# brdav/refign

Measured on AMD Instinct MI355X. Metric: image-pairs/s (align+seg fwd+bwd, 1080x1920), higher is better.
Workload: dtype bf16

## Files before the change

include/refign_hip.h:

```cpp
#ifndef REFIGN_HIP_H
#define REFIGN_HIP_H

#ifdef __cplusplus
extern "C" {
#endif

#define RFN_OK 0
#define RFN_EINVAL (-1)
#define RFN_ELAUNCH (-2)
#define RFN_ENOTSUP (-3)
#define RFN_ENONDET (-4)

#define RFN_ABI_VERSION 5

typedef void* rfn_stream_t;

int rfn_abi_version(void);
const char* rfn_last_error(void);

int rfn_set_deterministic(int on);
int rfn_get_deterministic(void);

int rfn_corr_fwd_f32(const float* in1, const float* in2, float* out, int B, int C, int iH, int iW,
                     int kH, int kW, int patchH, int patchW, int padH, int padW, int dilH, int dilW,
// ... 42 lines not shown
int rfn_maxpool2x2_nhwc16(const void* x, void* y, int B, int H, int W, int C, int dtype, rfn_stream_t stream);
int rfn_retile_copy(const void* src, void* dst, int B, int h, int w, int k, int units16, int src_stride16, int backward,
                    rfn_stream_t stream);

unsigned long rfn_refine_workspace_bytes(int B);
int rfn_refine_f32(const float* logits_trg, const float* logits_ref, const unsigned char* warp_mask,
                   const float* certs, float* out, void* workspace, int B, int C, int H, int W, float gamma,
                   int flags, rfn_stream_t stream);

int rfn_label_majority(const long* gt, long* out, int B, int H, int W, int scale, int n_classes, int ignore_index,
                       float min_ratio, rfn_stream_t stream);

int rfn_align_tail_f32(const float* logits_ref, const float* flow_q, const float* logvar_q, float* warped,
                       unsigned char* mask, float* cert, float* flow_up, int B, int C, int H, int W, int h,
                       int w, rfn_stream_t stream);

int rfn_dwconv3x3_nhwc_fwd(const void* x, const float* weight, const float* bias, void* y, int B, int H, int W,
                           int C, int dilation, int dtype, int flip, rfn_stream_t stream);
int rfn_dwconv3x3_nhwc_fwd_stats(const void* x, const float* weight, const float* bias, void* y, double* sums, int B, int H,
                                 int W, int C, int dilation, int dtype, rfn_stream_t stream);
int rfn_dwconv3x3_nhwc_stats(const void* x, const float* weight, const float* bias, double* sums, int B, int H, int W, int C,
                             int dilation, int dtype, rfn_stream_t stream);
int rfn_dwconv3x3_bn_act_nhwc_fwd(const void* x, const float* weight, const float* bias, const float* gamma, const float* beta,
                                  const double* sums, float* running_mean, float* running_var, void* y, int B, int H, int W,
                                  int C, int dilation, float eps, float momentum, int relu, int dtype, rfn_stream_t stream);

int rfn_dwconv3x3_gelu_nhwc_fwd(const void* x, const float* weight, const float* bias, void* y_pre, void* y_act, int B,
                                int H, int W, int C, int dtype, rfn_stream_t stream);
unsigned long rfn_dwconv3x3_bwd_weight_workspace_bytes(int C);
int rfn_dwconv3x3_nhwc_bwd_weight(const void* x, const void* grad_y, float* grad_weight, float* grad_bias,
// ... 302 lines not shown
```

refign_amd/csrc/bilinear.h:

```cpp
#pragma once
#include <hip/hip_runtime.h>

namespace rfn {

struct WarpTap {
  int o00, o01, o10, o11;
  float w00, w01, w10, w11;
  bool inside;
  float tx, ty;
  bool v00, v01, v10, v11;
  bool finite;
};

__device__ __forceinline__ WarpTap warp_tap(float gx, float gy, float fx, float fy, int H, int W) {
#pragma clang fp contract(off)
  const float wm = (float)max(W - 1, 1), hm = (float)max(H - 1, 1);
  const float vx = 2.0f * (gx + fx) / wm - 1.0f;
  const float vy = 2.0f * (gy + fy) / hm - 1.0f;
  const float ix = ((vx + 1.0f) / 2.0f) * (float)(W - 1);
  const float iy = ((vy + 1.0f) / 2.0f) * (float)(H - 1);
  float x0f = floorf(ix), y0f = floorf(iy);
  WarpTap t;
  t.tx = ix - x0f;
  t.ty = iy - y0f;
  x0f = fminf(fmaxf(x0f, -2.0f), (float)W);
  y0f = fminf(fmaxf(y0f, -2.0f), (float)H);
  if (!(ix == ix) || !(iy == iy)) { x0f = -2.0f; y0f = -2.0f; }
  const int x0 = (int)x0f, y0 = (int)y0f, x1 = x0 + 1, y1 = y0 + 1;
  const bool vx0 = x0 >= 0 && x0 < W, vx1 = x1 >= 0 && x1 < W;
  const bool vy0 = y0 >= 0 && y0 < H, vy1 = y1 >= 0 && y1 < H;
  const int cx0 = min(max(x0, 0), W - 1), cx1 = min(max(x1, 0), W - 1);
  const int cy0 = min(max(y0, 0), H - 1), cy1 = min(max(y1, 0), H - 1);
  t.o00 = cy0 * W + cx0; t.o01 = cy0 * W + cx1; t.o10 = cy1 * W + cx0; t.o11 = cy1 * W + cx1;
  t.v00 = vx0 && vy0; t.v01 = vx1 && vy0; t.v10 = vx0 && vy1; t.v11 = vx1 && vy1;
  const float ax = 1.0f - t.tx, ay = 1.0f - t.ty;
  t.w00 = t.v00 ? ax * ay : 0.0f;
  t.w01 = t.v01 ? t.tx * ay : 0.0f;
  t.w10 = t.v10 ? ax * t.ty : 0.0f;
  t.w11 = t.v11 ? t.tx * t.ty : 0.0f;
  t.inside = (vx > -1.0f) && (vy > -1.0f) && (vx < 1.0f) && (vy < 1.0f);
  t.finite = (ix == ix) && (iy == iy) && fabsf(ix) < 1e9f && fabsf(iy) < 1e9f;
  return t;
}

__device__ __forceinline__ float tap_sample(const float* __restrict__ src, const WarpTap& t) {
#pragma clang fp contract(off)
  return src[t.o00] * t.w00 + src[t.o01] * t.w01 + src[t.o10] * t.w10 + src[t.o11] * t.w11;
}

template <bool CLAMP>
__device__ __forceinline__ void up_split(float s, int in, int& i0, int& i1, float& l1) {
  if constexpr (CLAMP) {
    i0 = min((int)s, in - 1);
    i1 = i0 + (i0 < in - 1 ? 1 : 0);
  } else {
    i0 = (int)s;
    i1 = min(i0 + 1, in - 1);
  }
  l1 = s - (float)i0;
}
template <bool CLAMP = true>
__device__ __forceinline__ void up_src(int dst, float scale, int in, int& i0, int& i1, float& l1) {
  up_split<CLAMP>(fmaxf(scale * ((float)dst + 0.5f) - 0.5f, 0.f), in, i0, i1, l1);
}
__device__ __forceinline__ void up_src_nofma(int dst, float scale, int in, int& i0, int& i1, float& l1) {
  float s;
  {
#pragma clang fp contract(off)
    s = scale * ((float)dst + 0.5f) - 0.5f;
  }
  up_split<true>(fmaxf(s, 0.f), in, i0, i1, l1);
}

__device__ __forceinline__ void up_cell_window(int cell, float scale, int out_size, int& lo, int& hi) {
  const float inv = 1.f / scale;
  lo = cell <= 1 ? 0 : max(0, (int)floorf(((float)cell - 0.5f) * inv - 0.5f) - 1);
  hi = min(out_size, (int)ceilf(((float)cell + 1.5f) * inv - 0.5f) + 2);
}

}
```

refign_amd/csrc/refine.hip:

```cpp
#include "common.h"

namespace rfn {

constexpr int kClasses = 19;
constexpr int kPartials = 256;

__device__ __forceinline__ bool is_static_large(int c) {
  return (c <= 4) || (c >= 8 && c <= 10);
}

__global__ __launch_bounds__(256) void refine_entropy_kernel(const float* __restrict__ logits,
                                                             double* __restrict__ partials, int HW) {
  const int n = blockIdx.y;
  const float* p = logits + (size_t)n * kClasses * HW;
  double local = 0.0;
  for (int pix = blockIdx.x * 256 + threadIdx.x; pix < HW; pix += kPartials * 256) {
    float v[kClasses];
    float m = -INFINITY;
#pragma unroll
    for (int c = 0; c < kClasses; ++c) {
      v[c] = p[(size_t)c * HW + pix];
      m = fmaxf(m, v[c]);
    }
    float sum = 0.0f;
#pragma unroll
    for (int c = 0; c < kClasses; ++c) {
      v[c] -= m;
      sum += expf(v[c]);
    }
    const float lsum = logf(sum);
    float ent = 0.0f;
#pragma unroll
    for (int c = 0; c < kClasses; ++c) {
      const float lp = v[c] - lsum;
      ent -= (expf(v[c]) / sum) * lp;
    }
    local += (double)ent;
  }
  __shared__ double red[4];
#pragma unroll
  for (int o = 32; o > 0; o >>= 1) local += __shfl_xor(local, o, 64);
  if ((threadIdx.x & 63) == 0) red[threadIdx.x >> 6] = local;
  __syncthreads();
  if (threadIdx.x == 0) partials[(size_t)n * kPartials + blockIdx.x] = red[0] + red[1] + red[2] + red[3];
}

__global__ __launch_bounds__(256) void refine_blend_kernel(const float* __restrict__ lt, const float* __restrict__ lr,
                                                           const unsigned char* __restrict__ wmask,
                                                           const float* __restrict__ certs, float* __restrict__ out,
                                                           const double* __restrict__ partials, int HW, float gamma,
                                                           int flags) {
  const int n = blockIdx.y;
  __shared__ double red[4];
  __shared__ float s_trust;
  {
    double v = partials[(size_t)n * kPartials + threadIdx.x];
#pragma unroll
    for (int o = 32; o > 0; o >>= 1) v += __shfl_xor(v, o, 64);
    if ((threadIdx.x & 63) == 0) red[threadIdx.x >> 6] = v;
    __syncthreads();
    if (threadIdx.x == 0) {
      const double mean_ent = (red[0] + red[1] + red[2] + red[3]) / (double)HW;
      const float eta_mean = (float)(mean_ent / log((double)kClasses));
      s_trust = powf(eta_mean, gamma);
    }
    __syncthreads();
  }
  const float s = s_trust;
  const int pix = blockIdx.x * 256 + threadIdx.x;
  if (pix >= HW) return;
  const float* pt = lt + (size_t)n * kClasses * HW + pix;
  const float* pr = lr + (size_t)n * kClasses * HW + pix;
  float a[kClasses], b[kClasses];
  float ma = -INFINITY, mb = -INFINITY;
#pragma unroll
  for (int c = 0; c < kClasses; ++c) {
    a[c] = pt[(size_t)c * HW];
    b[c] = pr[(size_t)c * HW];
    ma = fmaxf(ma, a[c]);
    mb = fmaxf(mb, b[c]);
  }
  float sa = 0.0f, sb = 0.0f;
#pragma unroll
  for (int c = 0; c < kClasses; ++c) {
    a[c] = expf(a[c] - ma);
    b[c] = expf(b[c] - mb);
    sa += a[c];
    sb += b[c];
  }
  int ia = 0, ib = 0;
  float pa = -1.0f, pb = -1.0f;
#pragma unroll
  for (int c = 0; c < kClasses; ++c) {
    a[c] = a[c] / sa;
    b[c] = b[c] / sb;
    if (a[c] > pa) { pa = a[c]; ia = c; }
    if (b[c] > pb) { pb = b[c]; ib = c; }
  }
  const bool M = !(flags & 1) && is_static_large(ia) && is_static_large(ib);
  const float P = (certs != nullptr && !(flags & 2)) ? certs[(size_t)n * HW + pix] : 0.5f;
  const bool valid = (wmask == nullptr) || (wmask[(size_t)n * HW + pix] != 0);
  float* po = out + (size_t)n * kClasses * HW + pix;
#pragma unroll
  for (int c = 0; c < kClasses; ++c) {
    const float mc = (M && is_static_large(c)) ? 1.0f : 0.0f;
    const float eps = valid ? s * fmaxf(P, mc) : 0.0f;
    po[(size_t)c * HW] = (1.0f - eps) * a[c] + eps * b[c];
  }
}

__global__ __launch_bounds__(64) void label_majority_kernel(const long* __restrict__ gt, long* __restrict__ out, int H,
                                                            int W, int oh, int ow, int scale, int n_classes, int ignore,
                                                            float min_ratio) {
  const int cell = blockIdx.x, n = blockIdx.y, lane = threadIdx.x;
  const int cy = cell / ow, cx = cell % ow;
  const int y0 = cy * scale, x0 = cx * scale;
  const int hh = min(scale, H - y0), ww = min(scale, W - x0);
  const long* g = gt + (size_t)n * H * W;
  const int nb = n_classes + 1;
  int cnt[33];
#pragma unroll
  for (int c = 0; c < 33; ++c) cnt[c] = 0;
  for (int i = lane; i < hh * ww; i += 64) {
// ... 57 lines not shown
```

refign_amd/csrc/warp.hip:

```cpp
#include "bilinear.h"
#include "common.h"

namespace rfn {

template <int CG>
__global__ __launch_bounds__(256) void warp_kernel(const float* __restrict__ x, const float* __restrict__ flow,
                                                   float* __restrict__ out, unsigned char* __restrict__ mask,
                                                   int C, int H, int W) {
  const int pix = blockIdx.x * 256 + threadIdx.x;
  const int HW = H * W;
  if (pix >= HW) return;
  const int n = blockIdx.z, c0 = blockIdx.y * CG;
  const int gy = pix / W, gx = pix - gy * W;
  const float* fl = flow + (size_t)n * 2 * HW;
  const WarpTap t = warp_tap((float)gx, (float)gy, fl[pix], fl[HW + pix], H, W);
  if (mask != nullptr && blockIdx.y == 0) mask[(size_t)n * HW + pix] = t.inside ? 1 : 0;
  const float* src = x + ((size_t)n * C + c0) * HW;
  float* dst = out + ((size_t)n * C + c0) * HW + pix;
  const int cend = min(CG, C - c0);
  for (int c = 0; c < cend; ++c) dst[(size_t)c * HW] = tap_sample(src + (size_t)c * HW, t);
}

__device__ __forceinline__ int det_exponent(unsigned bits) { return max((int)(bits >> 23), 1) - 126; }
__device__ __forceinline__ double pow2(int e) { return __longlong_as_double((long long)(1023 + e) << 52); }
// ... 96 lines not shown
  const long idx = (long)blockIdx.x * 256 + threadIdx.x;
  if (idx < nx) {
    const unsigned mb = maxbits[idx / HW];
    float v = 0.0f;
    if (mb >= 0x7f800000u) v = __uint_as_float(0x7fc00000u);
    else if (mb != 0u) v = (float)((double)acc[idx] * pow2(det_exponent(mb) - F));
    gx_out[idx] = v;
  } else if (idx < nx + nf) {
    const long j = idx - nx;
    float s = 0.0f;
    for (int g = 0; g < G; ++g) s += part[(size_t)g * nf + j];
    gflow[j] = s;
  }
}

__device__ __forceinline__ float up_sample(const float* __restrict__ p, int w, int y0, int y1, int x0, int x1,
                                           float ly0, float ly1, float lx0, float lx1) {
#pragma clang fp contract(off)
  return ly0 * (lx0 * p[y0 * w + x0] + lx1 * p[y0 * w + x1]) + ly1 * (lx0 * p[y1 * w + x0] + lx1 * p[y1 * w + x1]);
}

__global__ __launch_bounds__(256) void align_tail_kernel(const float* __restrict__ logits,
                                                         const float* __restrict__ flow_q,
                                                         const float* __restrict__ logvar_q,
                                                         float* __restrict__ warped, unsigned char* __restrict__ mask,
                                                         float* __restrict__ cert, float* __restrict__ flow_up, int C,
                                                         int H, int W, int h, int w, float sy, float sx) {
  const int pix = blockIdx.x * 256 + threadIdx.x;
  const int HW = H * W, hw = h * w;
  if (pix >= HW) return;
  const int n = blockIdx.z;
  const int gy = pix / W, gx = pix - gy * W;
  int y0, y1, x0, x1;
  float ly1, lx1;
  up_src_nofma(gy, sy, h, y0, y1, ly1);
  up_src_nofma(gx, sx, w, x0, x1, lx1);
// ... 125 lines not shown
```

refign_amd/graphs.py:

```python
import contextlib
import gc
import os
import warnings

import torch


def enabled():
    return os.environ.get("RFN_HIP_GRAPH", "1") != "0"


def concurrent_stream(device, peers, priority=0, tries=8, spin_cycles=4_000_000):
    cur = torch.cuda.current_stream(device)

    def span(streams):
        start, end = torch.cuda.Event(enable_timing=True), torch.cuda.Event(enable_timing=True)
        start.record(cur)
        for st in streams:
            if st != cur:
                st.wait_event(start)
            with torch.cuda.stream(st):
                torch.cuda._sleep(spin_cycles)
        for st in streams:
            if st != cur:
# ... 40 lines not shown
    if isinstance(out, (list, tuple)):
        return type(out)(_fresh_containers(o) for o in out)
    return out


class GraphedNoGrad:
    def __init__(self, fn, name, warmup=1):
        self.fn, self.name, self.warmup = fn, name, warmup
        self.generation = 0
        self.states = {}

    def reset(self):
        self.generation += 1
        self.states.clear()

    def __call__(self, *tensors):
        if not tensors[0].is_cuda or not enabled() or torch.is_grad_enabled() or \
                torch.cuda.is_current_stream_capturing():
            return self.fn(*tensors)
        key = (tuple((tuple(t.shape), t.dtype, t.device) for t in tensors), torch.is_autocast_enabled("cuda"),
               torch.get_autocast_dtype("cuda"), self.generation)
        st = self.states.get(key)
        if st is None:
            st = self.states[key] = {"calls": 0, "graph": None, "failed": False}
        if st["failed"]:
            return self.fn(*tensors)
        if st["graph"] is None:
            st["calls"] += 1
            if st["calls"] <= self.warmup:
                return self.fn(*tensors)
            try:
                self._capture(st, tensors)
            except Exception as e:
                st["failed"] = True
                warnings.warn(f"refign_amd.graphs: capture of '{self.name}' failed ({type(e).__name__}: {e}); "
                              f"running it eagerly")
                torch.cuda.synchronize()
                return self.fn(*tensors)
        for s, t in zip(st["inputs"], tensors):
            s.copy_(t)
        st["graph"].replay()
        return _fresh_containers(st["outputs"])

    def _capture(self, st, tensors):
        inputs = [t.clone() for t in tensors]
        cur = torch.cuda.current_stream()
        side = torch.cuda.Stream()
        side.wait_stream(cur)
        with torch.cuda.stream(side):
            self.fn(*inputs)
        cur.wait_stream(side)
        torch.cuda.synchronize()
        g = torch.cuda.CUDAGraph()
        try:
            with _no_cyclic_gc(), torch.cuda.graph(g, capture_error_mode="thread_local"):
                outputs = self.fn(*inputs)
        except BaseException:
            torch.cuda.set_stream(cur)
            raise
        st["graph"], st["inputs"], st["outputs"] = g, inputs, outputs


class GraphedStep:

    def __init__(self, fn, name, warmup=2, shared=None, capture_context=None, after_capture=None, on_replay=None,
                 before_capture=None):
        self.fn, self.name, self.warmup = fn, name, warmup
        self.capture_context = capture_context
        self.after_capture, self.on_replay = after_capture, on_replay
        self.before_capture = before_capture
        self._last = None
# ... 307 lines not shown
```

refign_amd/refine.py:

```python
import torch

from . import _lib
from ._tensor import ptr, require_device_tensor, same_device


@torch.no_grad()
def refine(logits_trg, logits_ref, warp_mask, certs, gamma=0.25, disable_M=False, disable_P=False):
    logits_trg = require_device_tensor(logits_trg.float().contiguous(), "logits_trg", torch.float32)
    logits_ref = require_device_tensor(logits_ref.float().contiguous(), "logits_ref", torch.float32)
    dev = same_device(logits_trg, logits_ref, warp_mask, certs)
    B, C, H, W = logits_trg.shape
    assert C == 19, 'we assume cityscapes classes'
    if logits_ref.shape != logits_trg.shape:
        raise RuntimeError("refine: logits_trg / logits_ref shape mismatch")
    m8 = None
    if warp_mask is not None:
        if tuple(warp_mask.shape) != (B, H, W):
            raise RuntimeError("refine: warp_mask must be (B,H,W)")
        m8 = warp_mask.contiguous()
        m8 = m8.view(torch.uint8) if m8.dtype == torch.bool else m8.to(torch.uint8)
    if certs is not None:
        certs = require_device_tensor(certs.float().contiguous(), "certs", torch.float32)
        if certs.numel() != B * H * W:
            raise RuntimeError("refine: certs must be (B,1,H,W)")
    lib = _lib.load_library()
    ws = torch.empty(lib.rfn_refine_workspace_bytes(B), dtype=torch.uint8, device=dev)
    out = torch.empty_like(logits_trg)
    flags = (1 if disable_M else 0) | (2 if disable_P else 0)
    _lib.call("rfn_refine_f32", dev, ptr(logits_trg), ptr(logits_ref), ptr(m8), ptr(certs), ptr(out), ptr(ws), B, C, H, W,
              float(gamma), flags)
    return out
```

refign_amd/uda.py:

```python
import contextlib
import copy
import math
import os
import random
from typing import Optional, Sequence

import numpy as np
import torch
import torch.nn as nn
import torch.nn.functional as F

from . import align as align_mod
from . import refine as refine_mod
from ._tensor import const_tensor, upload_async
from . import dacs as _dacs
from . import f8 as _f8
from .graphs import GraphedNoGrad, GraphedSegment, GraphedSplitStep, GraphedStep
from .params import ema_update
from .upsample import interpolate_bilinear
from .config import instantiate_class
from . import seg as _seg
from .seg import DeviceBox, defer_logits, draw_crop_offsets, hrda_backbone, hrda_head, predraw_crop, push_device_crop

IMNET_MEAN = (0.485, 0.456, 0.406)
# ... 93 lines not shown

def _upsample_logits(logits, size):
    if logits.is_cuda:
        logits = logits.contiguous()
    return interpolate_bilinear(logits, size=size)


def _logits_for_loss(model, logits, size):
    return defer_logits(logits, size, _seg.fused_ce_consumer(model))


_ALIGN_PREFETCH = True
_MERGE_FD_BACKWARD = True
_EARLY_MIXED_FWD = True
_SRC_BWD_AFTER_TEACHER = True
_SIDE_PRIORITY = 0


class DomainAdaptationSegmentationModel(nn.Module):

    def __init__(self,
                 optimizer_init: dict,
                 lr_scheduler_init: dict,
                 backbone: nn.Module,
                 head: nn.Module,
                 loss: nn.Module,
                 alignment_backbone: Optional[nn.Module] = None,
                 alignment_head: Optional[nn.Module] = None,
                 metrics: dict = {},
                 backbone_lr_factor: float = 1.0,
# ... 395 lines not shown

    def _training_step_graphed(self, batch, images_src, gt_src, src_classes, opt, sch):
        ready = torch.cuda.current_stream().record_event() if self._overlap_teacher(images_src) else None
        off = self._crop_offsets(images_src, "src")
        cur = torch.cuda.current_stream()
        feat_next = self._take_imnet_prefetch(images_src) if self.enable_fdist else None
        src_graph, mix_graph = self._graphs["source_pass"], self._graphs["mixed_pass"]
        src_graph.forward(images_src, off, variant=feat_next is not None)
        src_fwd_done = cur.record_event()
        mix = early = None
        hold = _SRC_BWD_AFTER_TEACHER and ready is not None
        if hold:
            mix = self._mixed_stream(images_src)
            if mix is not None:
                mix.wait_event(ready)
            early = self._start_target_branch(batch, images_src, after=ready)
            if mix is not None:
                cur.wait_stream(self._side_stream)
        if feat_next is not None:
            feat_next = feat_next.clone()
            prefetch_free = cur.record_event()
            losses = src_graph.backward(images_src, gt_src, feat_next)
        else:
            losses = src_graph.backward(images_src, gt_src)
            prefetch_free = cur.record_event()
        if not hold:
            mix = self._mixed_stream(images_src) if ready is not None else None
            if mix is not None:
                mix.wait_event(ready)
            early = None if ready is None else self._start_target_branch(batch, images_src, after=ready)
        self.log("train_loss_src", losses[0])
        if self.enable_fdist:
            self.log("train_loss_featdist_src", losses[1])
        if early is None:
            mix = None
        run_on = cur if mix is None else mix
        if mix is not None and getattr(self, "_grad_buffer", None) is not None:
            self._grad_buffer.reduce_first_now()
        nb = batch['image_trg'].shape[0]
        src_nb, gt_nb = (images_src[:nb], gt_src[:nb]) if images_src.shape[0] > nb else (images_src, gt_src)
        early_fwd = (_EARLY_MIXED_FWD and mix is not None and self._dacs_kernels_usable(src_nb, early[0], gt_nb))
        if mix is not None:
            self.__dict__["_mixed_concurrent_steps"] = self.__dict__.get("_mixed_concurrent_steps", 0) + 1
            if early_fwd:
                mix.wait_event(src_fwd_done)
# ... 48 lines not shown
        if src_graph.any_failed() != mix_graph.any_failed():
            (mix_graph if src_graph.any_failed() else src_graph).give_up()
        opt.step()
        sch.step()
        self.global_step += 1

    def _prefetch_next(self, batch, prefetch_free, branch_done, with_flow, stream):
        nxt = batch.get("image_src_next")
        if nxt is not None:
            self.prefetch_imnet_features(nxt, after=prefetch_free, stream=stream)
        if batch.get("image_trg_next") is not None and batch.get("image_ref_next") is not None and with_flow \
                and self._next_step_aligns(batch["image_src"]):
            with torch.no_grad():
                self.prefetch_align_flow(batch["image_ref_next"], batch["image_trg_next"], after=branch_done, stream=stream)

    @torch.no_grad()
    def _target_branch(self, batch):
        if self.adapt_to_ref and random.random() < 0.5:
            adapt_to_ref, images_trg = True, batch['image_ref']
        else:
            adapt_to_ref, images_trg = False, batch['image_trg']
        if self.use_refign and not adapt_to_ref:
            return images_trg, self._teacher_align_refine(images_trg, batch['image_ref'])
        m_logits_trg = self.m_head(self._graphs["teacher_backbone"](images_trg))
        m_logits_trg = _upsample_logits(m_logits_trg, images_trg.shape[-2:])
        self.__dict__["_adapted_to_ref_steps"] = self.__dict__.get("_adapted_to_ref_steps", 0) + int(adapt_to_ref)
        return images_trg, F.softmax(m_logits_trg, dim=1)

    def _overlap_teacher(self, x):
        return x.is_cuda

    def _start_target_branch(self, batch, images_src, after=None):
        self._ensure_side_stream(images_src.device)
        if after is not None:
            self._side_stream.wait_event(after)
        else:
            if self.adapt_to_ref and self.use_hrda and self.training:
                H, W = images_src.shape[-2:]
                predraw_crop(H, W, (int(H * 0.5), int(W * 0.5)), self.hrda_output_stride * 2.0)
            self._side_stream.wait_stream(torch.cuda.current_stream())
        with torch.cuda.stream(self._side_stream):
            return self._target_branch(batch)

    def _ensure_side_stream(self, device):
        if getattr(self, "_side_stream", None) is None or self._side_stream.device != device:
            if _SIDE_PRIORITY == 0:
                from .graphs import concurrent_stream
                with torch.cuda.device(device):
                    self._side_stream, self._side_stream_probe = concurrent_stream(device, [torch.cuda.current_stream(device)])
                return
            self._side_stream = torch.cuda.Stream(device=device, priority=_SIDE_PRIORITY)

    def _teacher_align_refine(self, images_trg, images_ref):
        b = images_trg.shape[0]
        m_input = torch.cat((images_trg, images_ref))
        m_logits = self.m_head(self._graphs["teacher_backbone"](m_input))
        m_logits = _upsample_logits(m_logits, m_input.shape[-2:])
        m_logits_trg, m_logits_ref = torch.split(m_logits, [b, b], dim=0)
        if self.use_align:
            if self._align_split(images_trg):
                flow = self._take_align_prefetch(images_ref, images_trg)
                if flow is None:
                    flow = self._graphs["align_flow"](images_ref, images_trg)
                return self._graphs["tail_refine"](m_logits_trg.contiguous(), m_logits_ref.contiguous(), *flow)
            return self._graphs["align_refine"](m_logits_trg.contiguous(), m_logits_ref.contiguous(), images_ref,
                                                images_trg)
        return self.refine(m_logits_trg, m_logits_ref, None, None)

    def _align_refine(self, logits_trg, logits_ref, images_ref, images_trg):
        warped, warp_mask, warp_certs = self.align(logits_ref, images_ref, images_trg)
        return self.refine(logits_trg, warped, warp_mask, warp_certs)

    def _align_flow(self, images_ref, images_trg):
        return align_mod.align_flow(self.alignment_backbone, self.alignment_head, images_ref, images_trg)

    def _tail_refine(self, logits_trg, logits_ref, flow_q, logvar_q):
        warped, warp_mask, warp_certs = align_mod.align_from_flow(logits_ref, flow_q, logvar_q)
        return self.refine(logits_trg, warped, warp_mask, warp_certs)

    def _align_split(self, x):
        return _ALIGN_PREFETCH and self.use_refign and self.use_align and x.is_cuda and self._overlap_teacher(x)

    def _next_step_aligns(self, images_src):
        if not self.adapt_to_ref:
            return True
        state = random.getstate()
        try:
            if self.use_hrda:
                H, W = images_src.shape[-2:]
                draw_crop_offsets(H, W, (int(H * 0.5), int(W * 0.5)), self.hrda_output_stride * 2.0)
            return not random.random() < 0.5
# ... 198 lines not shown
                  'color_jitter_p': self.color_jitter_p, 'blur': random.uniform(0, 1) if self.blur else 0}
        classes = torch.unique(gt_src) if src_classes is None else src_classes
        bits = _dacs.draw_class_bits(classes, nb)
        jit, sig = [], []
        for i in range(nb):
            jit.append(_dacs.draw_jitter(self.color_jitter_s) if params['color_jitter'] > params['color_jitter_p']
                       else None)
            sig.append(np.random.uniform(0.15, 1.15) if params['blur'] > 0.5 else None)
        return {"bits": bits, "jitter": jit, "sigma": sig}

    def _dacs_kernels_usable(self, images_src, images_trg, gt_src):
        return os.environ.get("RFN_DACS_KERNEL", "1") != "0" and _dacs.usable(
            images_src, images_trg, gt_src, getattr(getattr(self, "head", None), "num_classes", 19))

    def _pseudo_labels(self, probs_trg):
        pseudo_prob, pseudo_label = torch.max(probs_trg, dim=1)
        weight = (pseudo_prob >= self.pseudo_label_threshold).sum() / pseudo_label.numel()
        pseudo_weight = torch.full_like(pseudo_prob, 1.0) * weight
        if self.psweight_ignore_top > 0:
            pseudo_weight[:, :self.psweight_ignore_top, :] = 0
        if self.psweight_ignore_bottom > 0:
            pseudo_weight[:, -self.psweight_ignore_bottom:, :] = 0
        return pseudo_label, pseudo_weight

    @torch.no_grad()
    def get_dacs_mix(self, images_trg, probs_trg, images_src, gt_src, src_classes=None):
        nb = images_trg.shape[0]
        if images_src.shape[0] > nb:
            images_src, gt_src = images_src[:nb], gt_src[:nb]
        cls = DomainAdaptationSegmentationModel
        if cls._dacs_kernels_usable(self, images_src, images_trg, gt_src):
# ... 131 lines not shown
```

Before: 17.48.

## Fuse teacher upsample, warp, refine and pseudo-label argmax into a low-res tail kernel

Adds a teacher-tail kernel pair that reads low-resolution teacher logits and flow directly. It bilinearly upsamples them on the fly, computes entropy-based trust, warps the reference logits, blends them and optionally emits only the per-pixel max probability and label. This avoids materialising full-resolution upsampled logits, warped logits and the full probability tensor before torch.max. The cost is more complex nested interpolation arithmetic per pixel and a risk of numerical differences from the original op order.

Result: no change. 17.62 (median of 6 runs) (+0.8%).

```diff
diff --git a/include/refign_hip.h b/include/refign_hip.h
--- a/include/refign_hip.h
+++ b/include/refign_hip.h
@@ -80,6 +80,11 @@
 int rfn_align_tail_f32(const float* logits_ref, const float* flow_q, const float* logvar_q, float* warped,
                        unsigned char* mask, float* cert, float* flow_up, int B, int C, int H, int W, int h,
                        int w, rfn_stream_t stream);
+
+int rfn_teacher_tail_f32(const float* logits_trg, const float* logits_ref, long stride_b, long stride_c, long stride_y,
+                         long stride_x, const float* flow_q, const float* logvar_q, void* workspace, float* probs,
+                         float* pseudo_prob, long* pseudo_label, unsigned char* mask, float* cert, int B, int C, int h, int w,
+                         int hf, int wf, int H, int W, float gamma, int flags, rfn_stream_t stream);
 
 int rfn_dwconv3x3_nhwc_fwd(const void* x, const float* weight, const float* bias, void* y, int B, int H, int W,
                            int C, int dilation, int dtype, int flip, rfn_stream_t stream);
diff --git a/refign_amd/csrc/bilinear.h b/refign_amd/csrc/bilinear.h
--- a/refign_amd/csrc/bilinear.h
+++ b/refign_amd/csrc/bilinear.h
@@ -10,6 +10,7 @@
   float tx, ty;
   bool v00, v01, v10, v11;
   bool finite;
+  int cx0, cx1, cy0, cy1;
 };
 
 __device__ __forceinline__ WarpTap warp_tap(float gx, float gy, float fx, float fy, int H, int W) {
@@ -31,6 +32,7 @@
   const bool vy0 = y0 >= 0 && y0 < H, vy1 = y1 >= 0 && y1 < H;
   const int cx0 = min(max(x0, 0), W - 1), cx1 = min(max(x1, 0), W - 1);
   const int cy0 = min(max(y0, 0), H - 1), cy1 = min(max(y1, 0), H - 1);
+  t.cx0 = cx0; t.cx1 = cx1; t.cy0 = cy0; t.cy1 = cy1;
   t.o00 = cy0 * W + cx0; t.o01 = cy0 * W + cx1; t.o10 = cy1 * W + cx0; t.o11 = cy1 * W + cx1;
   t.v00 = vx0 && vy0; t.v01 = vx1 && vy0; t.v10 = vx0 && vy1; t.v11 = vx1 && vy1;
   const float ax = 1.0f - t.tx, ay = 1.0f - t.ty;
@@ -43,9 +45,12 @@
   return t;
 }
 
+__device__ __forceinline__ float tap_combine(float nw, float ne, float sw, float se, const WarpTap& t) {
+#pragma clang fp contract(off)
+  return nw * t.w00 + ne * t.w01 + sw * t.w10 + se * t.w11;
+}
 __device__ __forceinline__ float tap_sample(const float* __restrict__ src, const WarpTap& t) {
-#pragma clang fp contract(off)
-  return src[t.o00] * t.w00 + src[t.o01] * t.w01 + src[t.o10] * t.w10 + src[t.o11] * t.w11;
+  return tap_combine(src[t.o00], src[t.o01], src[t.o10], src[t.o11], t);
 }
 
 template <bool CLAMP>
@@ -72,6 +77,15 @@
   up_split<true>(fmaxf(s, 0.f), in, i0, i1, l1);
 }
 
+__device__ __forceinline__ float up_lerp(float l0, float a, float l1, float b) {
+#pragma clang fp contract(off)
+  return l0 * a + l1 * b;
+}
+__device__ __forceinline__ float up_sample(const float* __restrict__ p, int w, int y0, int y1, int x0, int x1,
+                                           float ly0, float ly1, float lx0, float lx1) {
+  return up_lerp(ly0, up_lerp(lx0, p[y0 * w + x0], lx1, p[y0 * w + x1]), ly1, up_lerp(lx0, p[y1 * w + x0], lx1, p[y1 * w + x1]));
+}
+
 __device__ __forceinline__ void up_cell_window(int cell, float scale, int out_size, int& lo, int& hi) {
   const float inv = 1.f / scale;
   lo = cell <= 1 ? 0 : max(0, (int)floorf(((float)cell - 0.5f) * inv - 0.5f) - 1);
diff --git a/refign_amd/csrc/refine.hip b/refign_amd/csrc/refine.hip
--- a/refign_amd/csrc/refine.hip
+++ b/refign_amd/csrc/refine.hip
@@ -1,13 +1,7 @@
 #include "common.h"
+#include "refine_px.h"
 
 namespace rfn {
-
-constexpr int kClasses = 19;
-constexpr int kPartials = 256;
-
-__device__ __forceinline__ bool is_static_large(int c) {
-  return (c <= 4) || (c >= 8 && c <= 10);
-}
 
 __global__ __launch_bounds__(256) void refine_entropy_kernel(const float* __restrict__ logits,
                                                              double* __restrict__ partials, int HW) {
@@ -16,33 +10,11 @@
   double local = 0.0;
   for (int pix = blockIdx.x * 256 + threadIdx.x; pix < HW; pix += kPartials * 256) {
     float v[kClasses];
-    float m = -INFINITY;
 #pragma unroll
-    for (int c = 0; c < kClasses; ++c) {
-      v[c] = p[(size_t)c * HW + pix];
-      m = fmaxf(m, v[c]);
-    }
-    float sum = 0.0f;
-#pragma unroll
-    for (int c = 0; c < kClasses; ++c) {
-      v[c] -= m;
-      sum += expf(v[c]);
-    }
-    const float lsum = logf(sum);
-    float ent = 0.0f;
-#pragma unroll
-    for (int c = 0; c < kClasses; ++c) {
-      const float lp = v[c] - lsum;
-      ent -= (expf(v[c]) / sum) * lp;
-    }
-    local += (double)ent;
+    for (int c = 0; c < kClasses; ++c) v[c] = p[(size_t)c * HW + pix];
+    local += (double)pixel_entropy(v);
   }
-  __shared__ double red[4];
-#pragma unroll
-  for (int o = 32; o > 0; o >>= 1) local += __shfl_xor(local, o, 64);
-  if ((threadIdx.x & 63) == 0) red[threadIdx.x >> 6] = local;
-  __syncthreads();
-  if (threadIdx.x == 0) partials[(size_t)n * kPartials + blockIdx.x] = red[0] + red[1] + red[2] + red[3];
+  store_entropy_partial(local, partials, n);
 }
 
 __global__ __launch_bounds__(256) void refine_blend_kernel(const float* __restrict__ lt, const float* __restrict__ lr,
@@ -51,62 +23,23 @@
                                                            const double* __restrict__ partials, int HW, float gamma,
                                                            int flags) {
   const int n = blockIdx.y;
-  __shared__ double red[4];
-  __shared__ float s_trust;
-  {
-    double v = partials[(size_t)n * kPartials + threadIdx.x];
-#pragma unroll
-    for (int o = 32; o > 0; o >>= 1) v += __shfl_xor(v, o, 64);
-    if ((threadIdx.x & 63) == 0) red[threadIdx.x >> 6] = v;
-    __syncthreads();
-    if (threadIdx.x == 0) {
-      const double mean_ent = (red[0] + red[1] + red[2] + red[3]) / (double)HW;
-      const float eta_mean = (float)(mean_ent / log((double)kClasses));
-      s_trust = powf(eta_mean, gamma);
-    }
-    __syncthreads();
-  }
-  const float s = s_trust;
+  const float s = trust_score(partials, n, HW, gamma);
   const int pix = blockIdx.x * 256 + threadIdx.x;
   if (pix >= HW) return;
   const float* pt = lt + (size_t)n * kClasses * HW + pix;
   const float* pr = lr + (size_t)n * kClasses * HW + pix;
   float a[kClasses], b[kClasses];
-  float ma = -INFINITY, mb = -INFINITY;
 #pragma unroll
   for (int c = 0; c < kClasses; ++c) {
     a[c] = pt[(size_t)c * HW];
     b[c] = pr[(size_t)c * HW];
-    ma = fmaxf(ma, a[c]);
-    mb = fmaxf(mb, b[c]);
   }
-  float sa = 0.0f, sb = 0.0f;
-#pragma unroll
-  for (int c = 0; c < kClasses; ++c) {
-    a[c] = expf(a[c] - ma);
-    b[c] = expf(b[c] - mb);
-    sa += a[c];
-    sb += b[c];
-  }
-  int ia = 0, ib = 0;
-  float pa = -1.0f, pb = -1.0f;
-#pragma unroll
-  for (int c = 0; c < kClasses; ++c) {
-    a[c] = a[c] / sa;
-    b[c] = b[c] / sb;
-    if (a[c] > pa) { pa = a[c]; ia = c; }
-    if (b[c] > pb) { pb = b[c]; ib = c; }
-  }
-  const bool M = !(flags & 1) && is_static_large(ia) && is_static_large(ib);
   const float P = (certs != nullptr && !(flags & 2)) ? certs[(size_t)n * HW + pix] : 0.5f;
   const bool valid = (wmask == nullptr) || (wmask[(size_t)n * HW + pix] != 0);
+  refine_pixel(a, b, s, P, valid, flags);
   float* po = out + (size_t)n * kClasses * HW + pix;
 #pragma unroll
-  for (int c = 0; c < kClasses; ++c) {
-    const float mc = (M && is_static_large(c)) ? 1.0f : 0.0f;
-    const float eps = valid ? s * fmaxf(P, mc) : 0.0f;
-    po[(size_t)c * HW] = (1.0f - eps) * a[c] + eps * b[c];
-  }
+  for (int c = 0; c < kClasses; ++c) po[(size_t)c * HW] = a[c];
 }
 
 __global__ __launch_bounds__(64) void label_majority_kernel(const long* __restrict__ gt, long* __restrict__ out, int H,
diff --git a/refign_amd/csrc/refine_px.h b/refign_amd/csrc/refine_px.h
--- /dev/null
+++ b/refign_amd/csrc/refine_px.h
@@ -0,0 +1,92 @@
+#pragma once
+#include "common.h"
+
+namespace rfn {
+
+constexpr int kClasses = 19;
+constexpr int kPartials = 256;
+
+__device__ __forceinline__ bool is_static_large(int c) {
+  return (c <= 4) || (c >= 8 && c <= 10);
+}
+
+__device__ __forceinline__ float pixel_entropy(float (&v)[kClasses]) {
+  float m = -INFINITY;
+#pragma unroll
+  for (int c = 0; c < kClasses; ++c) m = fmaxf(m, v[c]);
+  float sum = 0.0f;
+#pragma unroll
+  for (int c = 0; c < kClasses; ++c) {
+    v[c] -= m;
+    sum += expf(v[c]);
+  }
+  const float lsum = logf(sum);
+  float ent = 0.0f;
+#pragma unroll
+  for (int c = 0; c < kClasses; ++c) {
+    const float lp = v[c] - lsum;
+    ent -= (expf(v[c]) / sum) * lp;
+  }
+  return ent;
+}
+
+__device__ __forceinline__ void store_entropy_partial(double local, double* __restrict__ partials, int n) {
+  __shared__ double red[4];
+#pragma unroll
+  for (int o = 32; o > 0; o >>= 1) local += __shfl_xor(local, o, 64);
+  if ((threadIdx.x & 63) == 0) red[threadIdx.x >> 6] = local;
+  __syncthreads();
+  if (threadIdx.x == 0) partials[(size_t)n * kPartials + blockIdx.x] = red[0] + red[1] + red[2] + red[3];
+}
+
+__device__ __forceinline__ float trust_score(const double* __restrict__ partials, int n, int HW, float gamma) {
+  __shared__ double red[4];
+  __shared__ float s_trust;
+  double v = partials[(size_t)n * kPartials + threadIdx.x];
+#pragma unroll
+  for (int o = 32; o > 0; o >>= 1) v += __shfl_xor(v, o, 64);
+  if ((threadIdx.x & 63) == 0) red[threadIdx.x >> 6] = v;
+  __syncthreads();
+  if (threadIdx.x == 0) {
+    const double mean_ent = (red[0] + red[1] + red[2] + red[3]) / (double)HW;
+    const float eta_mean = (float)(mean_ent / log((double)kClasses));
+    s_trust = powf(eta_mean, gamma);
+  }
+  __syncthreads();
+  return s_trust;
+}
+
+__device__ __forceinline__ void refine_pixel(float (&a)[kClasses], float (&b)[kClasses], float s, float P, bool valid, int flags) {
+  float ma = -INFINITY, mb = -INFINITY;
+#pragma unroll
+  for (int c = 0; c < kClasses; ++c) {
+    ma = fmaxf(ma, a[c]);
+    mb = fmaxf(mb, b[c]);
+  }
+  float sa = 0.0f, sb = 0.0f;
+#pragma unroll
+  for (int c = 0; c < kClasses; ++c) {
+    a[c] = expf(a[c] - ma);
+    b[c] = expf(b[c] - mb);
+    sa += a[c];
+    sb += b[c];
+  }
+  int ia = 0, ib = 0;
+  float pa = -1.0f, pb = -1.0f;
+#pragma unroll
+  for (int c = 0; c < kClasses; ++c) {
+    a[c] = a[c] / sa;
+    b[c] = b[c] / sb;
+    if (a[c] > pa) { pa = a[c]; ia = c; }
+    if (b[c] > pb) { pb = b[c]; ib = c; }
+  }
+  const bool M = !(flags & 1) && is_static_large(ia) && is_static_large(ib);
+#pragma unroll
+  for (int c = 0; c < kClasses; ++c) {
+    const float mc = (M && is_static_large(c)) ? 1.0f : 0.0f;
+    const float eps = valid ? s * fmaxf(P, mc) : 0.0f;
+    a[c] = (1.0f - eps) * a[c] + eps * b[c];
+  }
+}
+
+}
diff --git a/refign_amd/csrc/teachertail.hip b/refign_amd/csrc/teachertail.hip
--- /dev/null
+++ b/refign_amd/csrc/teachertail.hip
@@ -0,0 +1,271 @@
+#include "bilinear.h"
+#include "common.h"
+#include "refine_px.h"
+
+namespace rfn {
+
+constexpr int kTtT = 16;
+constexpr int kTtS = 20;
+constexpr int kTtF = 10;
+
+struct TtStrides {
+  long b, c, y, x;
+};
+
+constexpr int kTtGroups = 5;
+__device__ __forceinline__ constexpr int tt_group_first(int j) { return j < kTtGroups - 1 ? 4 * j : kClasses - 4; }
+typedef float tt_float4 __attribute__((ext_vector_type(4), aligned(4)));
+
+template <bool CL>
+__device__ __forceinline__ void tt_load4(const float* __restrict__ p, long sc, int c0, float (&v)[4]) {
+  if constexpr (CL) {
+    const tt_float4 q = *reinterpret_cast<const tt_float4*>(p + c0);
+    v[0] = q.x, v[1] = q.y, v[2] = q.z, v[3] = q.w;
+  } else {
+#pragma unroll
+    for (int k = 0; k < 4; ++k) v[k] = p[(c0 + k) * sc];
+  }
+}
+
+struct TtPixel {
+  float q[4][kTtGroups][4];
+  float ly0, ly1, lx0, lx1;
+};
+template <bool CL>
+__device__ __forceinline__ void tt_pixel_load(const float* __restrict__ p, const TtStrides& st, int pix, int W, int h, int w,
+                                              float sy, float sx, TtPixel& t) {
+  const long sc = CL ? 1 : st.c;
+  const int gy = pix / W, gx = pix - gy * W;
+  int y0, y1, x0, x1;
+  up_src(gy, sy, h, y0, y1, t.ly1);
+  up_src(gx, sx, w, x0, x1, t.lx1);
+  t.ly0 = 1.0f - t.ly1, t.lx0 = 1.0f - t.lx1;
+  const float* cell[4] = {p + y0 * st.y + x0 * st.x, p + y0 * st.y + x1 * st.x, p + y1 * st.y + x0 * st.x, p + y1 * st.y + x1 * st.x};
+#pragma unroll
+  for (int j = 0; j < kTtGroups; ++j)
+#pragma unroll
+    for (int i = 0; i < 4; ++i) tt_load4<CL>(cell[i], sc, tt_group_first(j), t.q[i][j]);
+}
+__device__ __forceinline__ void tt_pixel_blend(const TtPixel& t, float (&v)[kClasses]) {
+#pragma unroll
+  for (int j = 0; j < kTtGroups; ++j) {
+    const int c0 = tt_group_first(j);
+#pragma unroll
+    for (int k = 4 * j - c0; k < 4; ++k)
+      v[c0 + k] = up_lerp(t.ly0, up_lerp(t.lx0, t.q[0][j][k], t.lx1, t.q[1][j][k]), t.ly1,
+                          up_lerp(t.lx0, t.q[2][j][k], t.lx1, t.q[3][j][k]));
+  }
+}
+
+template <bool CL>
+__global__ __launch_bounds__(256) void tail_entropy_kernel(const float* __restrict__ lt, TtStrides st,
+                                                           double* __restrict__ partials, int H, int W, int h, int w,
+                                                           float sy, float sx) {
+  const int n = blockIdx.y, HW = H * W;
+  const float* p = lt + (size_t)n * st.b;
+  double local = 0.0;
+  for (long pix = blockIdx.x * 256 + threadIdx.x; pix < HW; pix += 2 * kPartials * 256) {
+    const long pix1 = pix + kPartials * 256;
+    const bool has1 = pix1 < HW;
+    TtPixel t0, t1;
+    tt_pixel_load<CL>(p, st, (int)pix, W, h, w, sy, sx, t0);
+    tt_pixel_load<CL>(p, st, has1 ? (int)pix1 : HW - 1, W, h, w, sy, sx, t1);
+    float v0[kClasses], v1[kClasses];
+    tt_pixel_blend(t0, v0);
+    tt_pixel_blend(t1, v1);
+    local += (double)pixel_entropy(v0);
+    const float e1 = pixel_entropy(v1);
+    local += has1 ? (double)e1 : 0.0;
+  }
+  store_entropy_partial(local, partials, n);
+}
+
+template <bool CL>
+__global__ __launch_bounds__(256) void tail_refine_kernel(const float* __restrict__ lt, const float* __restrict__ lr, TtStrides st,
+                                                          const float* __restrict__ flow_q, const float* __restrict__ logvar_q,
+                                                          const double* __restrict__ partials, float* __restrict__ probs,
+                                                          float* __restrict__ pseudo_prob, long* __restrict__ pseudo_label,
+                                                          unsigned char* __restrict__ mask, float* __restrict__ cert, int H, int W,
+                                                          int h, int w, int hf, int wf, float sy, float sx, float sfy, float sfx,
+                                                          float gamma, int flags) {
+  __shared__ __attribute__((aligned(16))) float lo[kTtF * kTtF * kTtS];
+  const int n = blockIdx.z, tid = threadIdx.x;
+  const int HW = H * W;
+  const long sc = CL ? 1 : st.c;
+  const float s = trust_score(partials, n, HW, gamma);
+
+  const int Y0 = blockIdx.y * kTtT, X0 = blockIdx.x * kTtT;
+  int fy0, fx0, nfy, nfx;
+  {
+    int i0, i1;
+    float l;
+    up_src(Y0, sy, h, fy0, i1, l);
+    up_src(min(Y0 + kTtT, H) - 1, sy, h, i0, i1, l);
+    nfy = min(i1 - fy0 + 1, kTtF);
+    up_src(X0, sx, w, fx0, i1, l);
+    up_src(min(X0 + kTtT, W) - 1, sx, w, i0, i1, l);
+    nfx = min(i1 - fx0 + 1, kTtF);
+  }
+  const float* pt = lt + (size_t)n * st.b;
+  for (int i = tid; i < nfy * nfx * kTtGroups; i += 256) {
+    const int q = i / kTtGroups, c0 = tt_group_first(i - q * kTtGroups);
+    const int fy = q / nfx, fx = q - fy * nfx;
+    float v[4];
+    tt_load4<CL>(pt + (fy0 + fy) * st.y + (fx0 + fx) * st.x, sc, c0, v);
+#pragma unroll
+    for (int k = 0; k < 4; ++k) lo[q * kTtS + c0 + k] = v[k];
+  }
+  __syncthreads();
+
+  const int gy = Y0 + tid / kTtT, gx = X0 + tid % kTtT;
+  if (gy >= H || gx >= W) return;
+  const int pix = gy * W + gx;
+
+  float P;
+  WarpTap t;
+  {
+    int y0, y1, x0, x1;
+    float ly1, lx1;
+    up_src_nofma(gy, sfy, hf, y0, y1, ly1);
+    up_src_nofma(gx, sfx, wf, x0, x1, lx1);
+    const float ly0 = 1.0f - ly1, lx0 = 1.0f - lx1;
+    const int hwf = hf * wf;
+    const float* fq = flow_q + (size_t)n * 2 * hwf;
+    const float fx = up_sample(fq, wf, y0, y1, x0, x1, ly0, ly1, lx0, lx1);
+    const float fy = up_sample(fq + hwf, wf, y0, y1, x0, x1, ly0, ly1, lx0, lx1);
+    const float lv = up_sample(logvar_q + (size_t)n * hwf, wf, y0, y1, x0, x1, ly0, ly1, lx0, lx1);
+    P = 1.0f - expf(-1.0f / (2.0f * expf(lv)));
+    t = warp_tap((float)gx, (float)gy, fx, fy, H, W);
+  }
+  if (cert != nullptr) cert[(size_t)n * HW + pix] = P;
+  if (mask != nullptr) mask[(size_t)n * HW + pix] = t.inside ? 1 : 0;
+  if (flags & 2) P = 0.5f;
+
+  float b[kClasses];
+  {
+    int ya0, ya1, yb0, yb1, xa0, xa1, xb0, xb1;
+    float lya1, lyb1, lxa1, lxb1;
+    up_src(t.cy0, sy, h, ya0, ya1, lya1);
+    up_src(t.cy1, sy, h, yb0, yb1, lyb1);
+    up_src(t.cx0, sx, w, xa0, xa1, lxa1);
+    up_src(t.cx1, sx, w, xb0, xb1, lxb1);
+    const float lya0 = 1.0f - lya1, lyb0 = 1.0f - lyb1, lxa0 = 1.0f - lxa1, lxb0 = 1.0f - lxb1;
+    const bool same_y = yb0 == ya0, same_x = xb0 == xa0;
+    const float* pr = lr + (size_t)n * st.b;
+    int cell[3][3];
+#pragma unroll
+    for (int j = 0; j < 3; ++j)
+#pragma unroll
+      for (int i = 0; i < 3; ++i) cell[j][i] = (int)(min(ya0 + j, h - 1) * st.y + min(xa0 + i, w - 1) * st.x);
+    float rr[2][3][3][4];
+#pragma unroll
+    for (int j = 0; j < 3; ++j)
+#pragma unroll
+      for (int i = 0; i < 3; ++i) tt_load4<CL>(pr + cell[j][i], sc, 0, rr[0][j][i]);
+#pragma unroll
+    for (int g = 0; g < kTtGroups; ++g) {
+      const int c0 = tt_group_first(g);
+      if (g + 1 < kTtGroups) {
+        if (g > 0)
+          asm volatile("" : "+v"(cell[0][0]), "+v"(cell[0][1]), "+v"(cell[0][2]), "+v"(cell[1][0]), "+v"(cell[1][1]), "+v"(cell[1][2]),
+                            "+v"(cell[2][0]), "+v"(cell[2][1]), "+v"(cell[2][2]), "+v"(b[tt_group_first(g - 1) + 3]));
+#pragma unroll
+        for (int j = 0; j < 3; ++j)
+#pragma unroll
+          for (int i = 0; i < 3; ++i) tt_load4<CL>(pr + cell[j][i], sc, tt_group_first(g + 1), rr[(g + 1) & 1][j][i]);
+      }
+      const auto& r = rr[g & 1];
+#pragma unroll
+      for (int k = 4 * g - c0; k < 4; ++k) {
+        float ha[3], hb[3];
+#pragma unroll
+        for (int j = 0; j < 3; ++j) {
+          ha[j] = up_lerp(lxa0, r[j][0][k], lxa1, r[j][1][k]);
+          hb[j] = up_lerp(lxb0, same_x ? r[j][0][k] : r[j][1][k], lxb1, same_x ? r[j][1][k] : r[j][2][k]);
+        }
+        const float nw = up_lerp(lya0, ha[0], lya1, ha[1]);
+        const float ne = up_lerp(lya0, hb[0], lya1, hb[1]);
+        const float sw = up_lerp(lyb0, same_y ? ha[0] : ha[1], lyb1, same_y ? ha[1] : ha[2]);
+        const float se = up_lerp(lyb0, same_y ? hb[0] : hb[1], lyb1, same_y ? hb[1] : hb[2]);
+        b[c0 + k] = tap_combine(nw, ne, sw, se, t);
+      }
+    }
+  }
+
+  float a[kClasses];
+  {
+    int y0, y1, x0, x1;
+    float ly1, lx1;
+    up_src(gy, sy, h, y0, y1, ly1);
+    up_src(gx, sx, w, x0, x1, lx1);
+    const float ly0 = 1.0f - ly1, lx0 = 1.0f - lx1;
+    const float* p00 = lo + ((y0 - fy0) * nfx + x0 - fx0) * kTtS;
+    const float* p01 = lo + ((y0 - fy0) * nfx + x1 - fx0) * kTtS;
+    const float* p10 = lo + ((y1 - fy0) * nfx + x0 - fx0) * kTtS;
+    const float* p11 = lo + ((y1 - fy0) * nfx + x1 - fx0) * kTtS;
+#pragma unroll
+    for (int c = 0; c < kClasses; ++c)
+      a[c] = up_lerp(ly0, up_lerp(lx0, p00[c], lx1, p01[c]), ly1, up_lerp(lx0, p10[c], lx1, p11[c]));
+  }
+
+  refine_pixel(a, b, s, P, t.inside, flags);
+
+  if (probs != nullptr) {
+    float* po = probs + (size_t)n * kClasses * HW + pix;
+#pragma unroll
+    for (int c = 0; c < kClasses; ++c) po[(size_t)c * HW] = a[c];
+  }
+  if (pseudo_prob != nullptr) {
+    float best = a[0];
+    int label = 0;
+#pragma unroll
+    for (int c = 1; c < kClasses; ++c) {
+      if (a[c] > best) {
+        best = a[c];
+        label = c;
+      }
+    }
+    pseudo_prob[(size_t)n * HW + pix] = best;
+    pseudo_label[(size_t)n * HW + pix] = (long)label;
+  }
+}
+
+}
+
+using namespace rfn;
+
+extern "C" {
+
+int rfn_teacher_tail_f32(const float* logits_trg, const float* logits_ref, long stride_b, long stride_c, long stride_y,
+                         long stride_x, const float* flow_q, const float* logvar_q, void* workspace, float* probs,
+                         float* pseudo_prob, long* pseudo_label, unsigned char* mask, float* cert, int B, int C, int h, int w,
+                         int hf, int wf, int H, int W, float gamma, int flags, rfn_stream_t stream) {
+  RFN_REQUIRE(logits_trg && logits_ref && flow_q && logvar_q && workspace, "rfn_teacher_tail_f32: null pointer");
+  RFN_REQUIRE(probs || pseudo_prob || mask || cert, "rfn_teacher_tail_f32: every output is NULL: nothing to compute");
+  RFN_REQUIRE((pseudo_prob == nullptr) == (pseudo_label == nullptr),
+              "rfn_teacher_tail_f32: pseudo_prob and pseudo_label come together");
+  RFN_REQUIRE(C == kClasses, "rfn_teacher_tail_f32: we assume cityscapes classes (C must be 19, got %d)", C);
+  RFN_REQUIRE(B > 0 && B <= 65535 && h > 0 && w > 0 && hf > 0 && wf > 0 && H > 0 && W > 0 && (long)H * W < 0x7fffffffL,
+              "rfn_teacher_tail_f32: bad size");
+  RFN_REQUIRE(2 * (long)h <= H && 2 * (long)w <= W,
+              "rfn_teacher_tail_f32: logits %d x %d -> %d x %d: up-sampling by at least 2 per axis expected", h, w, H, W);
+  RFN_REQUIRE(stride_b >= 0 && stride_c > 0 && stride_y > 0 && stride_x > 0, "rfn_teacher_tail_f32: non-positive stride");
+  RFN_REQUIRE((h - 1) * stride_y + (w - 1) * stride_x + (kClasses - 1) * stride_c < 0x7fffffffL,
+              "rfn_teacher_tail_f32: an image of the logits spans 2^31 elements or more");
+  RFN_REQUIRE(cdiv(H, kTtT) <= 65535, "rfn_teacher_tail_f32: image too tall");
+  hipStream_t s = (hipStream_t)stream;
+  const TtStrides st{stride_b, stride_c, stride_y, stride_x};
+  const float sy = (float)h / (float)H, sx = (float)w / (float)W;
+  const float sfy = (float)hf / (float)H, sfx = (float)wf / (float)W;
+  const bool cl = stride_c == 1;
+  const auto k1 = cl ? tail_entropy_kernel<true> : tail_entropy_kernel<false>;
+  hipLaunchKernelGGL(k1, dim3(kPartials, B), dim3(256), 0, s, logits_trg, st, (double*)workspace, H, W, h, w, sy, sx);
+  if (int rc = check_launch("tail_entropy_kernel")) return rc;
+  const auto k2 = cl ? tail_refine_kernel<true> : tail_refine_kernel<false>;
+  hipLaunchKernelGGL(k2, dim3(cdiv(W, kTtT), cdiv(H, kTtT), B), dim3(256), 0, s, logits_trg, logits_ref, st, flow_q, logvar_q,
+                     (const double*)workspace, probs, pseudo_prob, pseudo_label, mask, cert, H, W, h, w, hf, wf, sy, sx, sfy,
+                     sfx, gamma, flags);
+  return check_launch("tail_refine_kernel");
+}
+
+}
diff --git a/refign_amd/csrc/warp.hip b/refign_amd/csrc/warp.hip
--- a/refign_amd/csrc/warp.hip
+++ b/refign_amd/csrc/warp.hip
@@ -134,12 +134,6 @@
   }
 }
 
-__device__ __forceinline__ float up_sample(const float* __restrict__ p, int w, int y0, int y1, int x0, int x1,
-                                           float ly0, float ly1, float lx0, float lx1) {
-#pragma clang fp contract(off)
-  return ly0 * (lx0 * p[y0 * w + x0] + lx1 * p[y0 * w + x1]) + ly1 * (lx0 * p[y1 * w + x0] + lx1 * p[y1 * w + x1]);
-}
-
 __global__ __launch_bounds__(256) void align_tail_kernel(const float* __restrict__ logits,
                                                          const float* __restrict__ flow_q,
                                                          const float* __restrict__ logvar_q,
diff --git a/refign_amd/graphs.py b/refign_amd/graphs.py
--- a/refign_amd/graphs.py
+++ b/refign_amd/graphs.py
@@ -78,47 +78,48 @@
         self.generation += 1
         self.states.clear()
 
-    def __call__(self, *tensors):
+    def __call__(self, *tensors, static=()):
+        fn = (lambda *ts: self.fn(*ts, *static)) if static else self.fn
         if not tensors[0].is_cuda or not enabled() or torch.is_grad_enabled() or \
                 torch.cuda.is_current_stream_capturing():
-            return self.fn(*tensors)
+            return fn(*tensors)
         key = (tuple((tuple(t.shape), t.dtype, t.device) for t in tensors), torch.is_autocast_enabled("cuda"),
-               torch.get_autocast_dtype("cuda"), self.generation)
+               torch.get_autocast_dtype("cuda"), self.generation) + ((tuple(static),) if static else ())
         st = self.states.get(key)
         if st is None:
             st = self.states[key] = {"calls": 0, "graph": None, "failed": False}
         if st["failed"]:
-            return self.fn(*tensors)
+            return fn(*tensors)
         if st["graph"] is None:
             st["calls"] += 1
             if st["calls"] <= self.warmup:
-                return self.fn(*tensors)
+                return fn(*tensors)
             try:
-                self._capture(st, tensors)
+                self._capture(st, tensors, fn)
             except Exception as e:
                 st["failed"] = True
                 warnings.warn(f"refign_amd.graphs: capture of '{self.name}' failed ({type(e).__name__}: {e}); "
                               f"running it eagerly")
                 torch.cuda.synchronize()
-                return self.fn(*tensors)
+                return fn(*tensors)
         for s, t in zip(st["inputs"], tensors):
             s.copy_(t)
         st["graph"].replay()
         return _fresh_containers(st["outputs"])
 
-    def _capture(self, st, tensors):
+    def _capture(self, st, tensors, fn):
         inputs = [t.clone() for t in tensors]
         cur = torch.cuda.current_stream()
         side = torch.cuda.Stream()
         side.wait_stream(cur)
         with torch.cuda.stream(side):
-            self.fn(*inputs)
+            fn(*inputs)
         cur.wait_stream(side)
         torch.cuda.synchronize()
         g = torch.cuda.CUDAGraph()
         try:
             with _no_cyclic_gc(), torch.cuda.graph(g, capture_error_mode="thread_local"):
-                outputs = self.fn(*inputs)
+                outputs = fn(*inputs)
         except BaseException:
             torch.cuda.set_stream(cur)
             raise
diff --git a/refign_amd/refine.py b/refign_amd/refine.py
--- a/refign_amd/refine.py
+++ b/refign_amd/refine.py
@@ -30,3 +30,56 @@
     _lib.call("rfn_refine_f32", dev, ptr(logits_trg), ptr(logits_ref), ptr(m8), ptr(certs), ptr(out), ptr(ws), B, C, H, W,
               float(gamma), flags)
     return out
+
+
+class PseudoMax:
+
+    def __init__(self, prob, label):
+        self.prob, self.label = prob, label
+
+    def record_stream(self, stream):
+        self.prob.record_stream(stream)
+        self.label.record_stream(stream)
+
+
+@torch.no_grad()
+def refine_from_lowres(logits_trg, logits_ref, flow_q, logvar_q, size, gamma=0.25, disable_M=False, disable_P=False,
+                       output="probs", return_warp=False):
+    if output not in ("probs", "max"):
+        raise ValueError("refine_from_lowres: output is 'probs' or 'max'")
+    logits_trg, logits_ref = logits_trg.float(), logits_ref.float()
+    if logits_trg.dim() != 4 or logits_ref.shape != logits_trg.shape:
+        raise RuntimeError("refine_from_lowres: logits_trg / logits_ref must be (B,19,h,w), the same shape")
+    if not any(logits_trg.is_contiguous(memory_format=f) for f in (torch.channels_last, torch.contiguous_format)):
+        logits_trg = logits_trg.contiguous()
+    if logits_ref.stride() != logits_trg.stride():
+        logits_ref = torch.empty_like(logits_trg).copy_(logits_ref)
+    for t, name in ((logits_trg, "logits_trg"), (logits_ref, "logits_ref")):
+        if not t.is_cuda:
+            raise RuntimeError(f"{name} must be a HIP (cuda:N) tensor: refign_amd has no CPU path")
+    flow_q =require_device_tensor(flow_q.float().contiguous(), "flow_q", torch.float32)
+    logvar_q = require_device_tensor(logvar_q.float().contiguous(), "logvar_q", torch.float32)
+    dev = same_device(logits_trg, logits_ref, flow_q, logvar_q)
+    B, C, h, w = logits_trg.shape
+    assert C == 19, 'we assume cityscapes classes'
+    hf, wf = flow_q.shape[-2:]
+    if tuple(flow_q.shape) != (B, 2, hf, wf) or tuple(logvar_q.shape) != (B, 1, hf, wf):
+        raise RuntimeError("refine_from_lowres: flow_q must be (B,2,hf,wf) and logvar_q (B,1,hf,wf)")
+    H, W = int(size[0]), int(size[1])
+    sb, sc, sy, sx = logits_trg.stride()
+    lib = _lib.load_library()
+    ws = torch.empty(lib.rfn_refine_workspace_bytes(B), dtype=torch.uint8, device=dev)
+    probs = pmax = plabel = mask = cert = None
+    if output == "probs":
+        probs = torch.empty((B, C, H, W), dtype=torch.float32, device=dev)
+    else:
+        pmax = torch.empty((B, H, W), dtype=torch.float32, device=dev)
+        plabel = torch.empty((B, H, W), dtype=torch.int64, device=dev)
+    if return_warp:
+        mask = torch.empty((B, H, W), dtype=torch.uint8, device=dev)
+        cert = torch.empty((B, 1, H, W), dtype=torch.float32, device=dev)
+    flags = (1 if disable_M else 0) | (2 if disable_P else 0)
+    _lib.call("rfn_teacher_tail_f32", dev, ptr(logits_trg), ptr(logits_ref), sb, sc, sy, sx, ptr(flow_q), ptr(logvar_q), ptr(ws),
+              ptr(probs), ptr(pmax), ptr(plabel), ptr(mask), ptr(cert), B, C, h, w, hf, wf, H, W, float(gamma), flags)
+    out = probs if output == "probs" else PseudoMax(pmax, plabel)
+    return (out, mask.view(torch.bool), cert) if return_warp else out
diff --git a/refign_amd/uda.py b/refign_amd/uda.py
--- a/refign_amd/uda.py
+++ b/refign_amd/uda.py
@@ -131,6 +131,7 @@
 _MERGE_FD_BACKWARD = True
 _EARLY_MIXED_FWD = True
 _SRC_BWD_AFTER_TEACHER = True
+_TAIL_LOWRES = True
 _SIDE_PRIORITY = 0
 
 
@@ -556,7 +557,7 @@
             mix = self._mixed_stream(images_src)
             if mix is not None:
                 mix.wait_event(ready)
-            early = self._start_target_branch(batch, images_src, after=ready)
+            early = self._start_target_branch(batch, images_src, after=ready, pseudo=self._pseudo_tail(mix, batch, images_src, gt_src))
             if mix is not None:
                 cur.wait_stream(self._side_stream)
         if feat_next is not None:
@@ -570,7 +571,8 @@
             mix = self._mixed_stream(images_src) if ready is not None else None
             if mix is not None:
                 mix.wait_event(ready)
-            early = None if ready is None else self._start_target_branch(batch, images_src, after=ready)
+            early = None if ready is None else self._start_target_branch(
+                batch, images_src, after=ready, pseudo=self._pseudo_tail(mix, batch, images_src, gt_src))
         self.log("train_loss_src", losses[0])
         if self.enable_fdist:
             self.log("train_loss_featdist_src", losses[1])
@@ -649,14 +651,20 @@
             with torch.no_grad():
                 self.prefetch_align_flow(batch["image_ref_next"], batch["image_trg_next"], after=branch_done, stream=stream)
 
+    def _pseudo_tail(self, mix, batch, images_src, gt_src):
+        nb = batch['image_trg'].shape[0]
+        if not (_TAIL_LOWRES and _EARLY_MIXED_FWD and self._dacs_kernels_usable(images_src[:nb], batch['image_trg'], gt_src[:nb])):
+            return False
+        return True if mix is not None else None
+
     @torch.no_grad()
-    def _target_branch(self, batch):
+    def _target_branch(self, batch, pseudo=False):
         if self.adapt_to_ref and random.random() < 0.5:
             adapt_to_ref, images_trg = True, batch['image_ref']
         else:
             adapt_to_ref, images_trg = False, batch['image_trg']
         if self.use_refign and not adapt_to_ref:
-            return images_trg, self._teacher_align_refine(images_trg, batch['image_ref'])
+            return images_trg, self._teacher_align_refine(images_trg, batch['image_ref'], pseudo=pseudo)
         m_logits_trg = self.m_head(self._graphs["teacher_backbone"](images_trg))
         m_logits_trg = _upsample_logits(m_logits_trg, images_trg.shape[-2:])
         self.__dict__["_adapted_to_ref_steps"] = self.__dict__.get("_adapted_to_ref_steps", 0) + int(adapt_to_ref)
@@ -665,7 +673,7 @@
     def _overlap_teacher(self, x):
         return x.is_cuda
 
-    def _start_target_branch(self, batch, images_src, after=None):
+    def _start_target_branch(self, batch, images_src, after=None, pseudo=False):
         self._ensure_side_stream(images_src.device)
         if after is not None:
             self._side_stream.wait_event(after)
@@ -675,7 +683,7 @@
                 predraw_crop(H, W, (int(H * 0.5), int(W * 0.5)), self.hrda_output_stride * 2.0)
             self._side_stream.wait_stream(torch.cuda.current_stream())
         with torch.cuda.stream(self._side_stream):
-            return self._target_branch(batch)
+            return self._target_branch(batch, pseudo)
 
     def _ensure_side_stream(self, device):
         if getattr(self, "_side_stream", None) is None or self._side_stream.device != device:
@@ -686,11 +694,22 @@
                 return
             self._side_stream = torch.cuda.Stream(device=device, priority=_SIDE_PRIORITY)
 
-    def _teacher_align_refine(self, images_trg, images_ref):
+    def _teacher_align_refine(self, images_trg, images_ref, pseudo=False):
         b = images_trg.shape[0]
         m_input = torch.cat((images_trg, images_ref))
         m_logits = self.m_head(self._graphs["teacher_backbone"](m_input))
-        m_logits = _upsample_logits(m_logits, m_input.shape[-2:])
+        size = tuple(m_input.shape[-2:])
+        if _TAIL_LOWRES and self._align_split(images_trg) and m_logits.dtype == torch.float32 \
+                and 2 * m_logits.shape[-2] <= size[0] and 2 * m_logits.shape[-1] <= size[1]:
+            m_logits_trg, m_logits_ref = torch.split(m_logits, [b, b], dim=0)
+            flow = self._take_align_prefetch(images_ref, images_trg)
+            if flow is None:
+                flow = self._graphs["align_flow"](images_ref, images_trg)
+            if pseudo is None:
+                return self._tail_refine(m_logits_trg, m_logits_ref, *flow, size, "probs")
+            out = self._graphs["tail_refine"](m_logits_trg, m_logits_ref, *flow, static=(size, "max" if pseudo else "probs"))
+            return refine_mod.PseudoMax(*out) if pseudo else out
+        m_logits = _upsample_logits(m_logits, size)
         m_logits_trg, m_logits_ref = torch.split(m_logits, [b, b], dim=0)
         if self.use_align:
             if self._align_split(images_trg):
@@ -709,7 +728,11 @@
     def _align_flow(self, images_ref, images_trg):
         return align_mod.align_flow(self.alignment_backbone, self.alignment_head, images_ref, images_trg)
 
-    def _tail_refine(self, logits_trg, logits_ref, flow_q, logvar_q):
+    def _tail_refine(self, logits_trg, logits_ref, flow_q, logvar_q, size=None, output="probs"):
+        if size is not None:
+            out = refine_mod.refine_from_lowres(logits_trg, logits_ref, flow_q, logvar_q, size, gamma=self.gamma,
+                                                disable_M=self.disable_M, disable_P=self.disable_P, output=output)
+            return (out.prob, out.label) if output == "max" else out
         warped, warp_mask, warp_certs = align_mod.align_from_flow(logits_ref, flow_q, logvar_q)
         return self.refine(logits_trg, warped, warp_mask, warp_certs)
 
@@ -938,7 +961,10 @@
             images_src, images_trg, gt_src, getattr(getattr(self, "head", None), "num_classes", 19))
 
     def _pseudo_labels(self, probs_trg):
-        pseudo_prob, pseudo_label = torch.max(probs_trg, dim=1)
+        if isinstance(probs_trg, refine_mod.PseudoMax):
+            pseudo_prob, pseudo_label = probs_trg.prob, probs_trg.label
+        else:
+            pseudo_prob, pseudo_label = torch.max(probs_trg, dim=1)
         weight = (pseudo_prob >= self.pseudo_label_threshold).sum() / pseudo_label.numel()
         pseudo_weight = torch.full_like(pseudo_prob, 1.0) * weight
         if self.psweight_ignore_top > 0:
```
